# glacierbliss/iceberg_tracking_code

Measured on NVIDIA B200. Metric: tracked points/sec (24MP frame pairs, 20k pts, LK fwd+bwd+FB), higher is better.
Workload: dtype u8/int32 fixed point + f32 2x2 solve

## Files before the change

### iceberg_tracking_code_b200/csrc/common.cuh

```cuda
#pragma once
#include <cuda.h>
#include <cuda_runtime.h>
#include <stdint.h>
#include "../../include/ibt.h"

#define IBT_API extern "C" __attribute__((visibility("default")))

namespace ibt {

void set_last_error(cudaError_t e, const char *where);

inline int check_launch(const char *where)
{
    cudaError_t e = cudaGetLastError();
    if (e != cudaSuccess) { set_last_error(e, where); return IBT_E_CUDA; }
    return IBT_OK;
}

#define IBT_CUDA_TRY(expr)                                                        \
    do {                                                                          \
        cudaError_t e__ = (expr);                                                 \
        if (e__ != cudaSuccess) { ::ibt::set_last_error(e__, #expr); return IBT_E_CUDA; } \
    } while (0)

__host__ __device__ __noinline__ inline int r101_far(int i, int n)
{
    if (n == 1) return 0;
    const int p = 2 * (n - 1);
    i %= p;
    if (i < 0) i += p;
    return i < n ? i : p - i;
}
__host__ __device__ __forceinline__ int r101(int i, int n)
{
    if (i >= 0 && i < n) return i;
    if (i < 0) i = -i;
    if (i < n) return i;
    const int j = 2 * (n - 1) - i;
    if (j >= 0) return j;
    return r101_far(i, n);
}

#ifndef IBT_MBAR_SOFT
#define IBT_MBAR_SOFT 0
#endif
__device__ __forceinline__ void mbar_init(uint64_t *bar, int count)
{
    asm volatile("mbarrier.init.shared::cta.b64 [%0], %1;" ::"r"((unsigned)__cvta_generic_to_shared(bar)), "r"(count) : "memory");
}
__device__ __forceinline__ void mbar_expect_tx(uint64_t *bar, unsigned bytes)
{
    asm volatile("mbarrier.arrive.expect_tx.shared::cta.b64 _, [%0], %1;" ::"r"((unsigned)__cvta_generic_to_shared(bar)), "r"(bytes)
                 : "memory");
}
__device__ __forceinline__ void mbar_wait(uint64_t *bar, unsigned parity)
{
    const unsigned addr = (unsigned)__cvta_generic_to_shared(bar);
    for (int spin = 0; spin < (1 << 26); spin++) {
        unsigned ok;
        asm volatile("{\n .reg .pred p;\n mbarrier.try_wait.parity.shared::cta.b64 p, [%1], %2;\n selp.u32 %0, 1, 0, p;\n}"
                     : "=r"(ok) : "r"(addr), "r"(parity) : "memory");
        if (ok) return;
    }
    if (IBT_MBAR_SOFT) return;
    __trap();
}
__device__ __forceinline__ void tma_load_2d(void *smem_dst, const CUtensorMap *tmap, int c0, int c1, uint64_t *bar)
{
    asm volatile("cp.async.bulk.tensor.2d.shared::cluster.global.mbarrier::complete_tx::bytes [%0], [%1, {%2, %3}], [%4];"
                 ::"r"((unsigned)__cvta_generic_to_shared(smem_dst)), "l"(reinterpret_cast<uint64_t>(tmap)), "r"(c0), "r"(c1),
                 "r"((unsigned)__cvta_generic_to_shared(bar)) : "memory");
}
__device__ __forceinline__ void tma_prefetch_map(const CUtensorMap *tmap)
{
    asm volatile("prefetch.tensormap [%0];" ::"l"(reinterpret_cast<uint64_t>(tmap)) : "memory");
}
__device__ __forceinline__ void fence_proxy_async() { asm volatile("fence.proxy.async.shared::cta;" ::: "memory"); }

typedef CUresult (*EncodeTiledFn)(CUtensorMap *, CUtensorMapDataType, cuuint32_t, void *, const cuuint64_t *, const cuuint64_t *,
                                  const cuuint32_t *, const cuuint32_t *, CUtensorMapInterleave, CUtensorMapSwizzle,
                                  CUtensorMapL2promotion, CUtensorMapFloatOOBfill);
inline EncodeTiledFn encode_tiled_fn()
{
    static const EncodeTiledFn fn = [] {
        void *p = nullptr;
        cudaDriverEntryPointQueryResult q;
        EncodeTiledFn f = nullptr;
        if (cudaGetDriverEntryPoint("cuTensorMapEncodeTiled", &p, cudaEnableDefault, &q) == cudaSuccess &&
            q == cudaDriverEntryPointSuccess)
            f = reinterpret_cast<EncodeTiledFn>(p);
        (void)cudaGetLastError();
        return f;
    }();
    return fn;
}
inline bool make_map_2d(CUtensorMap *m, CUtensorMapDataType dt, const void *base, int cols, int rows, int64_t pitch_bytes,
                        int box_cols, int box_rows)
{
    EncodeTiledFn fn = encode_tiled_fn();
    if (!fn || reinterpret_cast<uintptr_t>(base) % 16 != 0 || pitch_bytes % 16 != 0 || box_cols > 256 || box_rows > 256) return false;
    const cuuint64_t gdim[2] = {(cuuint64_t)cols, (cuuint64_t)rows};
    const cuuint64_t gstride[1] = {(cuuint64_t)pitch_bytes};
    const cuuint32_t box[2] = {(cuuint32_t)box_cols, (cuuint32_t)box_rows};
    const cuuint32_t estr[2] = {1, 1};
    return fn(m, dt, 2, const_cast<void *>(base), gdim, gstride, box, estr, CU_TENSOR_MAP_INTERLEAVE_NONE,
              CU_TENSOR_MAP_SWIZZLE_NONE, CU_TENSOR_MAP_L2_PROMOTION_L2_128B, CU_TENSOR_MAP_FLOAT_OOB_FILL_NONE) == CUDA_SUCCESS;
}

__device__ __forceinline__ void pdl_wait() { asm volatile("griddepcontrol.wait;" ::: "memory"); }
__device__ __forceinline__ void pdl_launch_dependents() { asm volatile("griddepcontrol.launch_dependents;" ::: "memory"); }
template <typename... KArgs, typename... Args>
inline cudaError_t launch_pdl(void (*kernel)(KArgs...), dim3 grid, dim3 block, size_t smem, cudaStream_t st, Args... args)
{
    cudaLaunchConfig_t cfg = {};
    cfg.gridDim = grid; cfg.blockDim = block; cfg.dynamicSmemBytes = smem; cfg.stream = st;
    cudaLaunchAttribute attr[1];
    attr[0].id = cudaLaunchAttributeProgrammaticStreamSerialization;
    attr[0].val.programmaticStreamSerializationAllowed = 1;
// ... 37 lines not shown
```

### iceberg_tracking_code_b200/csrc/lk.cu

```cuda
#include "common.cuh"
#include <stdlib.h>
#include <string.h>
#include <type_traits>
#include <mutex>
#include <vector>

namespace ibt {

constexpr int LK_MARGIN = 3;

__host__ __device__ constexpr int lk_nl(int w) { return (w + 3) / 4; }
__host__ __device__ constexpr int lk_tcols(int w) { return 4 * lk_nl(w); }
__host__ __device__ constexpr int lk_ng0(int w, int h) { return (32 / lk_nl(w)) < h ? (32 / lk_nl(w)) : h; }
__host__ __device__ constexpr int lk_rg(int w, int h) { return (h + lk_ng0(w, h) - 1) / lk_ng0(w, h); }
__host__ __device__ constexpr int lk_ng(int w, int h) { return (h + lk_rg(w, h) - 1) / lk_rg(w, h); }
__host__ __device__ constexpr int lk_trows(int w, int h) { return lk_ng(w, h) * lk_rg(w, h); }
__host__ __device__ constexpr int lk_nstrips(int w) { return (lk_tcols(w) + 31) / 32; }
__host__ __device__ constexpr int lk_strip_cols(int w) { return (lk_tcols(w) + lk_nstrips(w) - 1) / lk_nstrips(w); }
__host__ __device__ constexpr bool lk_split(int w) { return w == 35; }
__host__ __device__ constexpr int lk_reach(int w) { return lk_split(w) ? lk_tcols(w) + 1 : (lk_nstrips(w) - 1) * lk_strip_cols(w) + 33; }
__host__ __device__ constexpr int lk_dpitch(int w) { return (lk_reach(w) + 6) & ~3; }
__host__ __device__ constexpr int lk_ipitch(int w) { return (15 + lk_reach(w) + 15) & ~15; }
__host__ __device__ constexpr int lk_jpitch(int w) { return (15 + 2 * LK_MARGIN + lk_tcols(w) + 4 + 15) & ~15; }

// ... 43 lines not shown
};

__device__ __forceinline__ long long warp_sum_wide(int v)
{
    const int lo = __reduce_add_sync(0xffffffffu, v & 0xffff);
    const int hi = __reduce_add_sync(0xffffffffu, v >> 16);
    return ((long long)hi << 16) + lo;
}

__device__ __forceinline__ int cv_floor(float v) { return __float2int_rd(v); }
__device__ __forceinline__ float no_nan(float v) { return v == v ? v : __int_as_float(0xff800000); }

__device__ __forceinline__ uint32_t dp2a_lo(uint32_t a, uint32_t b, uint32_t c)
{
    int d;
    asm("dp2a.lo.s32.u32 %0, %1, %2, %3;" : "=r"(d) : "r"(a), "r"(b), "r"((int)c));
    return (uint32_t)d;
}
__device__ __forceinline__ uint32_t dp2a_hi(uint32_t a, uint32_t b, uint32_t c)
{
    int d;
    asm("dp2a.hi.s32.u32 %0, %1, %2, %3;" : "=r"(d) : "r"(a), "r"(b), "r"((int)c));
    return (uint32_t)d;
}

__device__ __forceinline__ unsigned smem_u32(const void *p) { return (unsigned)__cvta_generic_to_shared(p); }
__device__ __forceinline__ void cp_async4(unsigned smem_dst, const void *gsrc)
{
    asm volatile("cp.async.ca.shared.global [%0], [%1], 4;" ::"r"(smem_dst), "l"(gsrc) : "memory");
}
__device__ __forceinline__ void cp_async4_zfill(unsigned smem_dst, const void *gsrc, int src_size)
{
    asm volatile("cp.async.ca.shared.global [%0], [%1], 4, %2;" ::"r"(smem_dst), "l"(gsrc), "r"(src_size) : "memory");
}
__device__ __forceinline__ void cp_async_commit() { asm volatile("cp.async.commit_group;" ::: "memory"); }
template <int N>
__device__ __forceinline__ void cp_async_wait() { asm volatile("cp.async.wait_group %0;" ::"n"(N) : "memory"); }

__device__ __forceinline__ void bilinear_weights(float a, float b, uint32_t &wtop, uint32_t &wbot,
                                                 int &iw00, int &iw01, int &iw10, int &iw11)
{
    const float oa = __fsub_rn(1.f, a), ob = __fsub_rn(1.f, b);
    iw00 = __float2int_rn(__fmul_rn(__fmul_rn(oa, ob), 16384.f));
    iw01 = __float2int_rn(__fmul_rn(__fmul_rn(a, ob), 16384.f));
    iw10 = __float2int_rn(__fmul_rn(__fmul_rn(oa, b), 16384.f));
    iw11 = 16384 - iw00 - iw01 - iw10;
    wtop = ((uint32_t)iw00 & 0xffffu) | ((uint32_t)iw01 << 16);
    wbot = ((uint32_t)iw10 & 0xffffu) | ((uint32_t)iw11 << 16);
}

__device__ __forceinline__ bool window_oob(int ix, int iy, int winW, int winH, int rows, int cols)
{
    return ix < -winW || ix >= cols || iy < -winH || iy >= rows;
}

__device__ __noinline__ void stage_bytes_border(const LKLevel &L, int x0a, int y0, int nrows, int pitch, uint8_t *dst, int lane)
{
    for (int c = lane; c < pitch; c += 32) {
        const uint8_t *s = L.img + r101(x0a + c, L.cols);
        uint8_t *d = dst + c;
        int r = 0;
        for (; r + 4 <= nrows; r += 4) {
            const uint8_t v0 = __ldg(s + (int64_t)r101(y0 + r, L.rows) * L.img_pitch);
            const uint8_t v1 = __ldg(s + (int64_t)r101(y0 + r + 1, L.rows) * L.img_pitch);
            const uint8_t v2 = __ldg(s + (int64_t)r101(y0 + r + 2, L.rows) * L.img_pitch);
            const uint8_t v3 = __ldg(s + (int64_t)r101(y0 + r + 3, L.rows) * L.img_pitch);
            d[r * pitch] = v0; d[(r + 1) * pitch] = v1; d[(r + 2) * pitch] = v2; d[(r + 3) * pitch] = v3;
        }
        for (; r < nrows; r++) d[r * pitch] = __ldg(s + (int64_t)r101(y0 + r, L.rows) * L.img_pitch);
    }
}

__device__ __forceinline__ void stage_bytes(const LKLevel &L, int x0a, int y0, int nrows, int pitch, int lane, uint8_t *dst)
{
    const bool interior = L.word_ok && x0a >= 0 && y0 >= 0 && y0 + nrows <= L.rows && x0a + pitch <= L.cols;
    if (interior) {
        const int ppw = pitch >> 2;
        const int rpp = 32 / ppw;
        const int sr = lane / ppw, sw = lane - sr * ppw;
        if (sr < rpp) {
            const uint8_t *src = L.img + (int64_t)(y0 + sr) * L.img_pitch + x0a + 4 * sw;
            unsigned d = smem_u32(dst) + sr * pitch + 4 * sw;
            const int64_t sstep = (int64_t)rpp * L.img_pitch;
            const int dstep = rpp * pitch;
#pragma unroll 4
            for (int r = sr; r < nrows; r += rpp) {
                cp_async4(d, src);
                src += sstep; d += dstep;
            }
        }
    } else {
        stage_bytes_border(L, x0a, y0, nrows, pitch, dst, lane);
    }
}

__device__ __forceinline__ bool patch_reflectable(int nx0, int nx1, int y0, int nrows, int rows, int cols)
{
    const int y1 = y0 + nrows - 1;
    return -nx0 <= nx1 && -nx0 < cols && 2 * (cols - 1) - nx1 >= nx0 && 2 * (cols - 1) - nx1 >= 0 &&
           -y0 <= y1 && -y0 < rows && 2 * (rows - 1) - y1 >= y0 && 2 * (rows - 1) - y1 >= 0;
}
__device__ __noinline__ void patch_reflect(uint8_t *patch, int pitch, int x0a, int nx0, int nx1, int y0, int nrows, int rows,
                                           int cols, int lane)
{
    __syncwarp();
    const int pw = pitch >> 2;
// ... 160 lines not shown
        a11[s] = a12[s] = a22[s] = c1[s] = c2[s] = 0;
        ipair[s] = 0; d00x[s] = d00y[s] = d01x[s] = d01y[s] = 0;
        const bool active = s < nstrips && lane < SC && s * SC + lane < winW;
        mtop[s] = active ? wtop : 0u; mbot[s] = active ? wbot : 0u;
        m00[s] = active ? iw00 : 0; m01[s] = active ? iw01 : 0; m10[s] = active ? iw10 : 0; m11[s] = active ? iw11 : 0;
        if (s < nstrips) {
            const uint8_t *ip = ip0 + s * SC + lane;
            const uint32_t *dp = dp0 + s * SC + lane;
            ipair[s] = (uint32_t)ip[0] | ((uint32_t)ip[1] << 8);
            const uint32_t dc = dp[0], dcr = dp[1];
            d00x[s] = (int)(short)(dc & 0xffffu); d00y[s] = (int)dc >> 16;
            d01x[s] = (int)(short)(dcr & 0xffffu); d01y[s] = (int)dcr >> 16;
        }
    }
#pragma unroll 4
    for (int r = 0; r < winH; r++) {
#pragma unroll
        for (int s = 0; s < NS; s++) {
            if (s < nstrips) {
                const int col = s * SC + lane;
                const uint8_t *ip = ip0 + (r + 1) * IP + col;
                const uint32_t *dp = dp0 + (r + 1) * DP + col;
                const uint32_t cpair = (uint32_t)ip[0] | ((uint32_t)ip[1] << 8);
                const uint32_t dc = dp[0], dcr = dp[1];
                const int d10x = (int)(short)(dc & 0xffffu), d10y = (int)dc >> 16;
                const int d11x = (int)(short)(dcr & 0xffffu), d11y = (int)dcr >> 16;
                uint32_t v = dp2a_lo(mtop[s], ipair[s], 256u);
                v = dp2a_lo(mbot[s], cpair, v);
                const int Iw = (int)(v >> 9);
                const int Ix = (d00x[s] * m00[s] + d01x[s] * m01[s] + d10x * m10[s] + d11x * m11[s] + 8192) >> 14;
                const int Iy = (d00y[s] * m00[s] + d01y[s] * m01[s] + d10y * m10[s] + d11y * m11[s] + 8192) >> 14;
                if ((SC >= 32 || lane < SC) && (NS * SC <= TC || col < TC))
                    tmpl_store(tmpl, r, TC, col, Ix, Iy);
                a11[s] += Ix * Ix; a12[s] += Ix * Iy; a22[s] += Iy * Iy;
                c1[s] += Iw * Ix; c2[s] += Iw * Iy;
                ipair[s] = cpair; d00x[s] = d10x; d00y[s] = d10y; d01x[s] = d11x; d01y[s] = d11y;
            }
        }
        __syncwarp();
    }
    for (int i = winH * TC + lane; i < TR * TC; i += 32) tmpl[i] = 0u;
    sA11 = sA12 = sA22 = sC1 = sC2 = 0;
#pragma unroll
    for (int s = 0; s < NS; s++) {
        if (s < nstrips) {
            sA11 += warp_sum_wide(a11[s]); sA12 += warp_sum_wide(a12[s]); sA22 += warp_sum_wide(a22[s]);
            sC1 += warp_sum_wide(c1[s]); sC2 += warp_sum_wide(c2[s]);
        }
    }
    __syncwarp();
}

template <int WW, int WH>
__device__ __forceinline__ void newton_sums(const LKArgs &a, const uint8_t *__restrict__ patch, int ox, int oy, uint32_t wtop,
                                            uint32_t wbot, const uint32_t *__restrict__ tmpl, int rowbase, int cq, bool lane_on,
                                            long long &S1, long long &S2)
{
    const int RG = (WW && WH) ? lk_rg(WW, WH) : a.rg;
    const int JP = WW ? lk_jpitch(WW) : a.jpitch, TC = WW ? lk_tcols(WW) : a.tcols;
    const uint32_t al = (uint32_t)ox & 3u;
    const uint32_t sel0 = 0x3210u + 0x1111u * al, sel1 = sel0 + 0x1111u;
    const uint32_t *jp = reinterpret_cast<const uint32_t *>(patch + (oy + rowbase) * JP + ((ox + 4 * cq) & ~3));
    const uint4 *tp = reinterpret_cast<const uint4 *>(tmpl + rowbase * TC + 4 * cq);
    uint32_t p0, p1;
    {
        const uint32_t w0 = jp[0], w1 = jp[1];
        p0 = __byte_perm(w0, w1, sel0); p1 = __byte_perm(w0, w1, sel1);
    }
    S1 = 0; S2 = 0;
    for (int r0 = 0; r0 < RG; r0 += 16) {
        const int r1 = (WW && WH) ? ((RG < r0 + 16) ? RG : r0 + 16) : min(RG, r0 + 16);
        uint32_t b1lo = 0, b1hi = 0, b2lo = 0, b2hi = 0;
#pragma unroll((WW && WH) ? 16 : 2)
        for (int r = r0; r < r1; r++) {
            jp += JP >> 2;
            const uint32_t w0 = jp[0], w1 = jp[1];
            const uint32_t c0 = __byte_perm(w0, w1, sel0), c1 = __byte_perm(w0, w1, sel1);
            const uint4 t = tp[r * (TC >> 2)];
            const uint32_t j0 = dp2a_lo(wbot, c0, dp2a_lo(wtop, p0, 256u)) >> 9;
            const uint32_t j1 = dp2a_lo(wbot, c1, dp2a_lo(wtop, p1, 256u)) >> 9;
            const uint32_t j2 = dp2a_hi(wbot, c0, dp2a_hi(wtop, p0, 256u)) >> 9;
            const uint32_t j3 = dp2a_hi(wbot, c1, dp2a_hi(wtop, p1, 256u)) >> 9;
            const uint32_t jb01 = __byte_perm(j0, j1, 0x5140u), jb23 = __byte_perm(j2, j3, 0x5140u);
            b1lo = dp2a_lo(t.y, jb23, dp2a_lo(t.x, jb01, b1lo));
            b1hi = dp2a_hi(t.y, jb23, dp2a_hi(t.x, jb01, b1hi));
            b2lo = dp2a_lo(t.w, jb23, dp2a_lo(t.z, jb01, b2lo));
            b2hi = dp2a_hi(t.w, jb23, dp2a_hi(t.z, jb01, b2hi));
            p0 = c0; p1 = c1;
        }
        if (!lane_on) { b1lo = b1hi = b2lo = b2hi = 0; }
        S1 += (long long)__reduce_add_sync(0xffffffffu, (int)b1lo) + ((long long)__reduce_add_sync(0xffffffffu, (int)b1hi) << 8);
        S2 += (long long)__reduce_add_sync(0xffffffffu, (int)b2lo) + ((long long)__reduce_add_sync(0xffffffffu, (int)b2hi) << 8);
    }
}

template <int WW, int WH>
__device__ __noinline__ long long window_err(const LKArgs &a, const uint8_t *jpatch, int ox, int oy, uint32_t wtop, uint32_t wbot,
                                             const uint8_t *ipatch, int iox, uint32_t iwtop, uint32_t iwbot, int rowbase, int cq,
                                             bool lane_on)
{
    const int winW = WW ? WW : a.winW, winH = WH ? WH : a.winH;
    const int RG = (WW && WH) ? lk_rg(WW, WH) : a.rg;
    const int JP = WW ? lk_jpitch(WW) : a.jpitch, IP = WW ? lk_ipitch(WW) : a.ipitch;
    const uint32_t jsel0 = 0x3210u + 0x1111u * ((uint32_t)ox & 3u), jsel1 = jsel0 + 0x1111u;
    const uint32_t isel0 = 0x3210u + 0x1111u * ((uint32_t)iox & 3u), isel1 = isel0 + 0x1111u;
    const uint32_t *jp = reinterpret_cast<const uint32_t *>(jpatch + (oy + rowbase) * JP + ((ox + 4 * cq) & ~3));
    const uint32_t *ip = reinterpret_cast<const uint32_t *>(ipatch + rowbase * IP + ((iox + 4 * cq) & ~3));
    uint32_t jp0 = __byte_perm(jp[0], jp[1], jsel0), jp1 = __byte_perm(jp[0], jp[1], jsel1);
    uint32_t ip0 = __byte_perm(ip[0], ip[1], isel0), ip1 = __byte_perm(ip[0], ip[1], isel1);
    long long S = 0;
    for (int r0 = 0; r0 < RG; r0 += 16) {
        int s = 0;
        for (int r = r0; r < min(RG, r0 + 16); r++) {
            jp += JP >> 2; ip += IP >> 2;
            const uint32_t jc0 = __byte_perm(jp[0], jp[1], jsel0), jc1 = __byte_perm(jp[0], jp[1], jsel1);
            const uint32_t ic0 = __byte_perm(ip[0], ip[1], isel0), ic1 = __byte_perm(ip[0], ip[1], isel1);
            if (rowbase + r < winH) {
                const int d0 = (int)(dp2a_lo(wbot, jc0, dp2a_lo(wtop, jp0, 256u)) >> 9) - (int)(dp2a_lo(iwbot, ic0, dp2a_lo(iwtop, ip0, 256u)) >> 9);
                const int d1 = (int)(dp2a_lo(wbot, jc1, dp2a_lo(wtop, jp1, 256u)) >> 9) - (int)(dp2a_lo(iwbot, ic1, dp2a_lo(iwtop, ip1, 256u)) >> 9);
                const int d2 = (int)(dp2a_hi(wbot, jc0, dp2a_hi(wtop, jp0, 256u)) >> 9) - (int)(dp2a_hi(iwbot, ic0, dp2a_hi(iwtop, ip0, 256u)) >> 9);
                const int d3 = (int)(dp2a_hi(wbot, jc1, dp2a_hi(wtop, jp1, 256u)) >> 9) - (int)(dp2a_hi(iwbot, ic1, dp2a_hi(iwtop, ip1, 256u)) >> 9);
                const int c = 4 * cq;
                if (c < winW) s += abs(d0);
                if (c + 1 < winW) s += abs(d1);
                if (c + 2 < winW) s += abs(d2);
                if (c + 3 < winW) s += abs(d3);
            }
            jp0 = jc0; jp1 = jc1; ip0 = ic0; ip1 = ic1;
        }
        if (!lane_on) s = 0;
        S += warp_sum_wide(s);
    }
    return S;
}

template <typename T>
__device__ __forceinline__ T *lk_chan(T *p, int c, int stride)
{
    using B = std::conditional_t<std::is_const<T>::value, const unsigned char, unsigned char>;
    return reinterpret_cast<T *>(reinterpret_cast<B *>(p) + (size_t)c * stride);
}

template <int WW, int WH, int CN>
__device__ __forceinline__ void lk_point(const LKPyr *PI, const LKPyr *PJ, int cn_rt, const LKArgs &a, float ptx, float pty,
                                         bool use_init, bool want_status, bool want_err, float &ox, float &oy, int &status,
                                         float &err, int &iters, unsigned char *slab, int rowbase, int cq, bool lane_on,
                                         int lane, const CUtensorMap *mapI, const CUtensorMap *mapJ, const CUtensorMap *mapD,
                                         uint64_t *bars, unsigned &phases)
{
    const float FLT_SCALE = 1.f / (1 << 20);
    const int cn = CN ? CN : cn_rt;
    const int winW = WW ? WW : a.winW, winH = WH ? WH : a.winH;
    const int IPITCH = WW ? lk_ipitch(WW) : a.ipitch, JPITCH = WW ? lk_jpitch(WW) : a.jpitch;
    const int DPITCH = WW ? lk_dpitch(WW) : a.dpitch;
    const int JROWS = winH + 1 + 2 * LK_MARGIN;
    const float halfx = (winW - 1) * 0.5f, halfy = (winH - 1) * 0.5f;
    uint32_t *tmpl = reinterpret_cast<uint32_t *>(slab);
    uint32_t *dpatch = reinterpret_cast<uint32_t *>(slab);
    uint8_t *ipatch = slab + a.off_ipatch;
    uint8_t *jpatch = slab + a.off_jpatch;
    auto ch = [&](auto *p, int c) { return lk_chan(p, c, a.warp_smem); };
    auto chl = [](const LKLevel &l, int c) -> const LKLevel & { return *lk_chan(&l, c, (int)sizeof(LKPyr)); };
    status = 1; err = 0.f;
    const int L = PI[0].nlevels;
    for (int level = L - 1; level >= 0; --level) {
        const LKLevel &LI = PI[0].lv[level];
        const LKLevel &LJ = PJ[0].lv[level];
        const int rows = LI.rows, cols = LI.cols;
        const float sc = __int_as_float((127 - level) << 23);
        float ppx = __fmul_rn(ptx, sc), ppy = __fmul_rn(pty, sc);
        float nx, ny;
        if (level == L - 1) {
            if (use_init) { nx = __fmul_rn(ox, sc); ny = __fmul_rn(oy, sc); }
            else { nx = ppx; ny = ppy; }
        } else { nx = __fmul_rn(ox, 2.f); ny = __fmul_rn(oy, 2.f); }
        ox = nx; oy = ny;

        ppx = __fsub_rn(ppx, halfx); ppy = __fsub_rn(ppy, halfy);
        const int ipx = cv_floor(no_nan(ppx)), ipy = cv_floor(no_nan(ppy));
        if (window_oob(ipx, ipy, winW, winH, rows, cols)) {
            if (level == 0) { status = 0; err = 0.f; }
            continue;
        }
        nx = no_nan(__fsub_rn(nx, halfx)); ny = no_nan(__fsub_rn(ny, halfy));

        const bool i_in = ipx >= 0 && ipy >= 0 && ipx + winW < cols && ipy + winH < rows;
        const bool i_fix = !i_in && patch_reflectable(ipx, ipx + winW, ipy, winH + 1, rows, cols);
        const bool i_tma = LI.tma_img && (i_in || i_fix), d_tma = LI.tma_der != 0;
        const int ipxa = i_tma ? (ipx & ~15) : (ipx & ~3);
        const int doff = d_tma ? (ipx & 3) : 0;
        int px0 = 0, py0 = 0, vx0 = 0;
        bool staged = false, j_tma = false, j_fix = false;
        const int jnx = cv_floor(nx), jny = cv_floor(ny);
        const bool j_ok = !window_oob(jnx, jny, winW, winH, rows, cols);
        if (j_ok) {
            const int bx = jnx - LK_MARGIN, by = jny - LK_MARGIN;
            const bool j_in = bx >= 0 && by >= 0 && bx + winW + 2 * LK_MARGIN < cols && by + JROWS <= rows;
            j_fix = !j_in && patch_reflectable(bx, bx + winW + 2 * LK_MARGIN, by, JROWS, rows, cols);
            j_tma = LJ.tma_img && (j_in || j_fix);
            px0 = j_tma ? (bx & ~15) : (bx & ~3); py0 = by; vx0 = bx;
            staged = true;
        }
        if (lane == 0 && (i_tma || d_tma || j_tma)) {
            fence_proxy_async();
            if (i_tma || d_tma) {
                mbar_expect_tx(&bars[0], (i_tma ? (unsigned)(IPITCH * (winH + 1)) : 0u) + (d_tma ? (unsigned)(DPITCH * 4 * (winH + 1)) : 0u));
                if (i_tma) tma_load_2d(ipatch, &mapI[level], ipxa, ipy, &bars[0]);
                if (d_tma) tma_load_2d(dpatch, &mapD[level], ipx - doff, ipy, &bars[0]);
            }
            if (j_tma) {
                mbar_expect_tx(&bars[1], (unsigned)(JPITCH * JROWS));
                tma_load_2d(jpatch, &mapJ[level], px0, py0, &bars[1]);
            }
        }
        for (int c = 0; c < cn; c++) {
            if (!i_tma) stage_bytes(chl(LI, c), ipxa, ipy, winH + 1, IPITCH, lane, ch(ipatch, c));
            if (!d_tma) stage_deriv<WW, WH>(chl(LI, c), a, ipx, ipy, ch(dpatch, c), lane);
        }
        cp_async_commit();
        if (j_ok && !j_tma)
            for (int c = 0; c < cn; c++) stage_bytes(chl(LJ, c), px0, py0, JROWS, JPITCH, lane, ch(jpatch, c));
        cp_async_commit();
        cp_async_wait<1>();
        if (i_tma || d_tma) { mbar_wait(&bars[0], phases & 1u); phases ^= 1u; }
        __syncwarp();
        if (i_tma && i_fix) patch_reflect(ipatch, IPITCH, ipxa, ipx, ipx + winW, ipy, winH + 1, rows, cols, lane);

        uint32_t wtop, wbot;
        int iw00, iw01, iw10, iw11;
        bilinear_weights(__fsub_rn(ppx, (float)ipx), __fsub_rn(ppy, (float)ipy), wtop, wbot, iw00, iw01, iw10, iw11);
        const uint32_t iwtop = wtop, iwbot = wbot;

        long long sA11, sA12, sA22, sC1, sC2;
        build_template<WW, WH>(a, ipatch + (ipx - ipxa), dpatch + doff, tmpl, wtop, wbot, iw00, iw01, iw10, iw11, lane,
                               sA11, sA12, sA22, sC1, sC2);
        for (int c = 1; c < cn; c++) {
            long long t11, t12, t22, tc1, tc2;
            build_template<WW, WH>(a, ch(ipatch, c) + (ipx - ipxa), ch(dpatch, c) + doff, ch(tmpl, c), wtop, wbot, iw00, iw01, iw10, iw11, lane,
                                   t11, t12, t22, tc1, tc2);
            sA11 += t11; sA12 += t12; sA22 += t22; sC1 += tc1; sC2 += tc2;
        }
        cp_async_wait<0>();
        if (j_tma) { mbar_wait(&bars[1], (phases >> 1) & 1u); phases ^= 2u; }
        __syncwarp();
        if (j_tma && j_fix) patch_reflect(jpatch, JPITCH, px0, vx0, vx0 + winW + 2 * LK_MARGIN, py0, JROWS, rows, cols, lane);
        const float A11 = __fmul_rn(__ll2float_rn(sA11), FLT_SCALE);
        const float A12 = __fmul_rn(__ll2float_rn(sA12), FLT_SCALE);
        const float A22 = __fmul_rn(__ll2float_rn(sA22), FLT_SCALE);
        float D = __fsub_rn(__fmul_rn(A11, A22), __fmul_rn(A12, A12));
        const float dA = __fsub_rn(A11, A22);
        const float disc = __fadd_rn(__fmul_rn(dA, dA), __fmul_rn(__fmul_rn(4.f, A12), A12));
        const float minEig = __fdiv_rn(__fsub_rn(__fadd_rn(A22, A11), __fsqrt_rn(disc)), (float)(2 * winW * winH));
        if (a.flags & IBT_LK_GET_MIN_EIGENVALS) err = minEig;
        if (minEig < a.minEigThr || D < 1.1920929e-07f) {
            if (level == 0) status = 0;
            continue;
        }
        D = __fdiv_rn(1.f, D);
        float pdx = 0.f, pdy = 0.f;
        for (int j = 0; j < a.maxCount; j++) {
            const int inx = cv_floor(nx), iny = cv_floor(ny);
            if (window_oob(inx, iny, winW, winH, rows, cols)) {
                if (level == 0) status = 0;
                break;
            }
            if (!staged || (unsigned)(inx - vx0) > 2u * LK_MARGIN || (unsigned)(iny - py0) > 2u * LK_MARGIN) {
                vx0 = inx - LK_MARGIN; px0 = vx0 & ~3; py0 = iny - LK_MARGIN;
                for (int c = 0; c < cn; c++) restage_sync(chl(LJ, c), px0, py0, JROWS, JPITCH, ch(jpatch, c), lane);
                staged = true;
            }
            bilinear_weights(__fsub_rn(nx, (float)inx), __fsub_rn(ny, (float)iny), wtop, wbot, iw00, iw01, iw10, iw11);
            long long sb1 = 0, sb2 = 0;
            for (int c = 0; c < cn; c++) {
                long long t1, t2;
                newton_sums<WW, WH>(a, ch(jpatch, c), inx - px0, iny - py0, wtop, wbot, ch(tmpl, c), rowbase, cq, lane_on, t1, t2);
                sb1 += t1; sb2 += t2;
            }
            ++iters;
            const float b1 = __fmul_rn(__ll2float_rn(sb1 - sC1), FLT_SCALE);
            const float b2 = __fmul_rn(__ll2float_rn(sb2 - sC2), FLT_SCALE);
            const float dx = __fmul_rn(__fsub_rn(__fmul_rn(A12, b2), __fmul_rn(A22, b1)), D);
            const float dy = __fmul_rn(__fsub_rn(__fmul_rn(A12, b1), __fmul_rn(A11, b2)), D);
            nx = __fadd_rn(nx, dx); ny = __fadd_rn(ny, dy);
            ox = __fadd_rn(nx, halfx); oy = __fadd_rn(ny, halfy);
            if (__fadd_rn(__fmul_rn(dx, dx), __fmul_rn(dy, dy)) <= a.eps2) break;
            if (j > 0 && fabsf(__fadd_rn(dx, pdx)) < 0.01f && fabsf(__fadd_rn(dy, pdy)) < 0.01f) {
                ox = __fsub_rn(ox, __fmul_rn(dx, 0.5f)); oy = __fsub_rn(oy, __fmul_rn(dy, 0.5f));
                break;
            }
            pdx = dx; pdy = dy;
        }
        if (status && level == 0 && !(a.flags & IBT_LK_GET_MIN_EIGENVALS) && (want_status || want_err)) {
            const float qx = __fsub_rn(ox, halfx), qy = __fsub_rn(oy, halfy);
            const int iqx = cv_floor(no_nan(qx)), iqy = cv_floor(no_nan(qy));
            if (window_oob(iqx, iqy, winW, winH, rows, cols)) { status = 0; err = 0.f; continue; }
            if (!want_err) continue;
            if (!staged || (unsigned)(iqx - vx0) > 2u * LK_MARGIN || (unsigned)(iqy - py0) > 2u * LK_MARGIN) {
                vx0 = iqx - LK_MARGIN; px0 = vx0 & ~3; py0 = iqy - LK_MARGIN;
                for (int c = 0; c < cn; c++) restage_sync(chl(LJ, c), px0, py0, JROWS, JPITCH, ch(jpatch, c), lane);
            }
            bilinear_weights(__fsub_rn(qx, (float)iqx), __fsub_rn(qy, (float)iqy), wtop, wbot, iw00, iw01, iw10, iw11);
            long long s = 0;
            for (int c = 0; c < cn; c++)
                s += window_err<WW, WH>(a, ch(jpatch, c), iqx - px0, iqy - py0, wtop, wbot, ch(ipatch, c), ipx - ipxa, iwtop, iwbot,
                                        rowbase, cq, lane_on);
            err = __fdiv_rn(__ll2float_rn(s), (float)(32 * winW * cn * winH));
        }
        __syncwarp();
    }
    cp_async_wait<0>();
    if (!status && !(a.flags & IBT_LK_GET_MIN_EIGENVALS)) err = 0.f;
}

template <int CN> using LKFrames = std::conditional_t<CN == 1, LKMaps, LKMcPyr>;

template <int WW, int WH, int CN>
__global__ void __launch_bounds__(256, CN == 1 ? 3 : 0)
lk_kernel(const __grid_constant__ LKArgs a, const __grid_constant__ LKFrames<CN> fr)
{
    extern __shared__ __align__(128) unsigned char lk_smem[];
    __shared__ __align__(8) uint64_t lk_bars[8][2];
    const int lane = threadIdx.x & 31, wib = threadIdx.x >> 5;
    if (lane == 0) {
        mbar_init(&lk_bars[wib][0], 1); mbar_init(&lk_bars[wib][1], 1);
        asm volatile("fence.mbarrier_init.release.cluster;" ::: "memory");
    }
    __syncwarp();
    unsigned phases = 0u;
    int cn = 1;
    if constexpr (CN != 1) cn = fr.cn;
    unsigned char *slab = lk_smem + (size_t)wib * a.warp_smem * cn;
    const int NL = WW ? lk_nl(WW) : a.nl, NG = (WW && WH) ? lk_ng(WW, WH) : a.ng, RG = (WW && WH) ? lk_rg(WW, WH) : a.rg;
    const int grp = lane / NL;
    const bool lane_on = grp < NG;
    const int rowbase = lane_on ? grp * RG : 0, cq = lane_on ? lane - grp * NL : 0;

  for (;;) {
    int k = 0;
    if (lane == 0) k = (int)atomicAdd(a.work_counter, 1u);
    k = __shfl_sync(0xffffffffu, k, 0);
    if (k >= a.n) break;
    if (a.alive && !a.alive[k]) continue;
    const float p0x = a.p0[2 * k], p0y = a.p0[2 * k + 1];
    float ptx = p0x, pty = p0y;
    int it_f = 0, it_b = 0;
    const int npass = a.fb ? 2 : 1;
    for (int pass = 0; pass < npass; ++pass) {
        float ox = 0.f, oy = 0.f, err;
        int status, iters = 0;
        const bool use_init = pass == 0 && (a.flags & IBT_LK_USE_INITIAL_FLOW) != 0;
        if (use_init) { ox = a.p1[2 * k]; oy = a.p1[2 * k + 1]; }
        const bool want_status = pass == 0 ? a.st1 != nullptr : a.st0 != nullptr;
        const bool want_err = pass == 0 ? a.err1 != nullptr : a.err0 != nullptr;
        const LKPyr *PI = a.pyr + pass, *PJ = a.pyr + (pass ^ 1);
        const CUtensorMap *mapI = nullptr, *mapJ = nullptr, *mapD = nullptr;
        if constexpr (CN == 1) { mapI = fr.imgI[pass]; mapJ = fr.imgJ[pass ^ 1]; mapD = fr.der[pass]; }
        else { PI = pass ? fr.J : fr.I; PJ = pass ? fr.I : fr.J; }
        lk_point<WW, WH, CN>(PI, PJ, cn, a, ptx, pty, use_init, want_status, want_err, ox, oy, status, err, iters,
                             slab, rowbase, cq, lane_on, lane, mapI, mapJ, mapD, lk_bars[wib], phases);
        if (pass == 0) it_f = iters; else it_b = iters;
        if (lane == 0) {
            if (pass == 0) {
                a.p1[2 * k] = ox; a.p1[2 * k + 1] = oy;
                if (a.st1) a.st1[k] = (uint8_t)status;
                if (a.err1) a.err1[k] = err;
            } else {
                if (a.p0r) { a.p0r[2 * k] = ox; a.p0r[2 * k + 1] = oy; }
                if (a.st0) a.st0[k] = (uint8_t)status;
                if (a.err0) a.err0[k] = err;
                const float d = hypotf(fabsf(__fsub_rn(p0x, ox)), fabsf(__fsub_rn(p0y, oy)));
                if (a.fbdist) a.fbdist[k] = d;
                if (a.alive) a.alive[k] = (d < a.fb_thresh) ? 1 : 0;
            }
        }
        ptx = ox; pty = oy;
    }
    if (lane == 0) {
        if (a.iters) {
            if (a.fb) { a.iters[2 * k] = it_f; a.iters[2 * k + 1] = it_b; }
            else a.iters[k] = it_f;
        }
        if (a.iter_total) atomicAdd(a.iter_total, (unsigned long long)(it_f + it_b));
    }
    __syncwarp();
  }
    if (lane == 0) {
        __threadfence();
        if (atomicAdd(a.work_counter + 1, 1u) == a.total_warps - 1u) {
            a.work_counter[0] = 0u; a.work_counter[1] = 0u;
            __threadfence();
        }
    }
}

static int fill_pyr(const ibt_pyramid_t *p, LKPyr &o, bool need_deriv)
{
    if (!p || p->nlevels < 1 || p->nlevels > IBT_MAX_LEVELS) return IBT_E_INVALID;
    o.nlevels = p->nlevels;
    for (int l = 0; l < p->nlevels; l++) {
        if (!p->img[l] || p->rows[l] <= 0 || p->cols[l] <= 0 || p->img_pitch[l] < p->cols[l] ||
            p->img_pitch[l] > 0x7fffffff)
            return IBT_E_INVALID;
        if (need_deriv && (!p->deriv[l] || p->deriv_pitch[l] % 4 != 0 || p->deriv_pitch[l] < (int64_t)p->cols[l] * 4 ||
                           reinterpret_cast<uintptr_t>(p->deriv[l]) % 4 != 0))
            return IBT_E_INVALID;
        o.lv[l].img = p->img[l];
        o.lv[l].deriv = reinterpret_cast<const uint32_t *>(p->deriv[l]);
        o.lv[l].img_pitch = (int)p->img_pitch[l];
        o.lv[l].deriv_pitch = (int)(p->deriv_pitch[l] / 4);
        o.lv[l].rows = p->rows[l];
        o.lv[l].cols = p->cols[l];
        o.lv[l].word_ok = (reinterpret_cast<uintptr_t>(p->img[l]) % 4 == 0) && (p->img_pitch[l] % 4 == 0);
        o.lv[l].tma_img = o.lv[l].tma_der = 0;
    }
    return IBT_OK;
}

struct LKQueue { int dev; cudaStream_t stream; unsigned int *words; };
static std::mutex lk_mu;
static int lk_max_ctas_per_sm = 0;
static std::vector<LKQueue> lk_queues;
static bool lk_attr_set[64] = {false};

static int lk_queue_for(int dev, cudaStream_t st, unsigned int **out)
{
    for (const LKQueue &q : lk_queues)
        if (q.dev == dev && q.stream == st) { *out = q.words; return IBT_OK; }
    unsigned int *w = nullptr;
    IBT_CUDA_TRY(cudaMalloc(&w, 2 * sizeof(unsigned int)));
    IBT_CUDA_TRY(cudaMemsetAsync(w, 0, 2 * sizeof(unsigned int), st));
    lk_queues.push_back({dev, st, w});
    *out = w;
    return IBT_OK;
}

static int launch_lk(LKArgs &a, const ibt_pyramid_t *const *A, const ibt_pyramid_t *const *B, int cn, bool planes, int winW,
                     int winH, int max_count, double epsilon, double min_eig, cudaStream_t st)
{
// ... 51 lines not shown
    if (epsilon > 10) epsilon = 10;
    a.eps2 = (float)(epsilon * epsilon);
    a.minEigThr = (float)min_eig;
    const size_t per_warp = (size_t)a.warp_smem * cn;
    const int max_warps = planes ? 16 : 24;
    int wpc = 1, best = 0, best_ctas = 1;
    for (int w = 1; w <= 8; w++) {
        const size_t per_cta = per_warp * w + 1024;
        if (per_cta > 200 * 1024) break;
        int ctas = (int)((227 * 1024) / per_cta);
        if (ctas > 32) ctas = 32;
        if (ctas * w > max_warps) ctas = max_warps / w;
        const int warps = ctas * w;
        if (warps >= best) { best = warps; wpc = w; best_ctas = ctas; }
    }
    if (best == 0) return IBT_E_INVALID;
    {
        std::lock_guard<std::mutex> lock(lk_mu);
        if (lk_max_ctas_per_sm > 0 && best_ctas > lk_max_ctas_per_sm) best_ctas = lk_max_ctas_per_sm;
    }
    const size_t smem = per_warp * wpc;
    void (*kern)(const LKArgs, const LKMaps) = lk_kernel<0, 0, 1>;
    if (winW == 21 && winH == 21) kern = lk_kernel<21, 21, 1>;
    else if (winW == 31 && winH == 31) kern = lk_kernel<31, 31, 1>;
    else if (winW == 35 && winH == 35) kern = lk_kernel<35, 35, 1>;
    int dev_id = 0;
    IBT_CUDA_TRY(cudaGetDevice(&dev_id));
    if (dev_id < 0 || dev_id >= 64) return IBT_E_INVALID;
    {
        std::lock_guard<std::mutex> lock(lk_mu);
        if (!lk_attr_set[dev_id]) {
            const int lim = 200 * 1024;
            IBT_CUDA_TRY(cudaFuncSetAttribute(lk_kernel<0, 0, 1>, cudaFuncAttributeMaxDynamicSharedMemorySize, lim));
            IBT_CUDA_TRY(cudaFuncSetAttribute(lk_kernel<21, 21, 1>, cudaFuncAttributeMaxDynamicSharedMemorySize, lim));
            IBT_CUDA_TRY(cudaFuncSetAttribute(lk_kernel<31, 31, 1>, cudaFuncAttributeMaxDynamicSharedMemorySize, lim));
            IBT_CUDA_TRY(cudaFuncSetAttribute(lk_kernel<35, 35, 1>, cudaFuncAttributeMaxDynamicSharedMemorySize, lim));
            IBT_CUDA_TRY(cudaFuncSetAttribute(lk_kernel<0, 0, 0>, cudaFuncAttributeMaxDynamicSharedMemorySize, lim));
            lk_attr_set[dev_id] = true;
        }
        const int rc = lk_queue_for(dev_id, st, &a.work_counter);
        if (rc) return rc;
    }
    int blocks = kNumSMs * best_ctas;
    const int need = (a.n + wpc - 1) / wpc;
    if (blocks > need) blocks = need;
    a.total_warps = (unsigned)(blocks * wpc);
    if (planes) lk_kernel<0, 0, 0><<<blocks, wpc * 32, smem, st>>>(a, mc);
    else kern<<<blocks, wpc * 32, smem, st>>>(a, maps);
    return check_launch(planes ? "ibt_lk_multichannel" : "ibt_lk");
}

}

IBT_API int ibt_lk_set_max_ctas_per_sm(int ctas)
{
    if (ctas < 0) return IBT_E_INVALID;
    std::lock_guard<std::mutex> lock(ibt::lk_mu);
    ibt::lk_max_ctas_per_sm = ctas;
    return IBT_OK;
}

IBT_API int ibt_lk(const ibt_pyramid_t *pyrI, const ibt_pyramid_t *pyrJ, const float *pts, float *next_pts, int N,
                   int winW, int winH, int max_count, double epsilon, double min_eig_threshold, int flags,
                   uint8_t *status, float *err, int32_t *iters, void *stream)
{
    ibt::LKArgs a;
    memset(&a, 0, sizeof(a));
    a.p0 = pts; a.n = N; a.flags = flags; a.fb = 0;
    a.p1 = next_pts; a.st1 = status; a.err1 = err; a.iters = iters;
    return ibt::launch_lk(a, &pyrI, &pyrJ, 1, false, winW, winH, max_count, epsilon, min_eig_threshold,
                          static_cast<cudaStream_t>(stream));
}

IBT_API int ibt_lk_fb(const ibt_pyramid_t *prev, const ibt_pyramid_t *next, const float *p0, int N, int winW, int winH,
                      int max_count, double epsilon, double min_eig_threshold, float fb_threshold, float *p1,
                      uint8_t *st1, float *err1, float *p0r, uint8_t *st0, float *err0, float *fbdist, uint8_t *alive,
                      int32_t *iters, unsigned long long *iter_total, void *stream)
{
    ibt::LKArgs a;
    memset(&a, 0, sizeof(a));
    a.p0 = p0; a.n = N; a.flags = 0; a.fb = 1; a.fb_thresh = fb_threshold;
    a.p1 = p1; a.st1 = st1; a.err1 = err1; a.p0r = p0r; a.st0 = st0; a.err0 = err0;
    a.fbdist = fbdist; a.alive = alive; a.iters = iters; a.iter_total = iter_total;
    return ibt::launch_lk(a, &prev, &next, 1, false, winW, winH, max_count, epsilon, min_eig_threshold,
                          static_cast<cudaStream_t>(stream));
}

IBT_API int ibt_lk_multichannel(const ibt_pyramid_t *const *pyrI, const ibt_pyramid_t *const *pyrJ, int cn, const float *pts,
                                float *next_pts, int N, int winW, int winH, int max_count, double epsilon,
                                double min_eig_threshold, int flags, uint8_t *status, float *err, int32_t *iters, void *stream)
{
    ibt::LKArgs a;
    memset(&a, 0, sizeof(a));
    a.p0 = pts; a.n = N; a.flags = flags; a.fb = 0;
    a.p1 = next_pts; a.st1 = status; a.err1 = err; a.iters = iters;
    return ibt::launch_lk(a, pyrI, pyrJ, cn, true, winW, winH, max_count, epsilon, min_eig_threshold,
                          static_cast<cudaStream_t>(stream));
}

IBT_API int ibt_lk_fb_multichannel(const ibt_pyramid_t *const *prev, const ibt_pyramid_t *const *next, int cn, const float *p0,
                                   int N, int winW, int winH, int max_count, double epsilon, double min_eig_threshold,
                                   float fb_threshold, float *p1, uint8_t *st1, float *err1, float *p0r, uint8_t *st0,
                                   float *err0, float *fbdist, uint8_t *alive, int32_t *iters, unsigned long long *iter_total,
                                   void *stream)
{
    if (cn < 2 || cn > ibt::LK_MC_MAX) return IBT_E_INVALID;
// ... 9 lines not shown
```

Before: 27.47 million.

## Skip per-iteration bounds checks when staged J patch is safe, add phase profiling

```diff
diff --git a/iceberg_tracking_code_b200/csrc/common.cuh b/iceberg_tracking_code_b200/csrc/common.cuh
--- a/iceberg_tracking_code_b200/csrc/common.cuh
+++ b/iceberg_tracking_code_b200/csrc/common.cuh
@@ -64,6 +64,20 @@
     }
     if (IBT_MBAR_SOFT) return;
     __trap();
+}
+__device__ __forceinline__ unsigned mbar_wait_parked(uint64_t *bar, unsigned parity)
+{
+    const unsigned addr = (unsigned)__cvta_generic_to_shared(bar);
+#pragma unroll 1
+    for (unsigned spin = 1; spin <= (1u << 20); spin++) {
+        unsigned ok;
+        asm volatile("{\n .reg .pred p;\n mbarrier.try_wait.parity.shared::cta.b64 p, [%1], %2, %3;\n selp.u32 %0, 1, 0, p;\n}"
+                     : "=r"(ok) : "r"(addr), "r"(parity), "r"(20000u) : "memory");
+        if (ok) return spin;
+    }
+    if (IBT_MBAR_SOFT) return 0u;
+    __trap();
+    return 0u;
 }
 __device__ __forceinline__ void tma_load_2d(void *smem_dst, const CUtensorMap *tmap, int c0, int c1, uint64_t *bar)
 {
diff --git a/iceberg_tracking_code_b200/csrc/lk.cu b/iceberg_tracking_code_b200/csrc/lk.cu
--- a/iceberg_tracking_code_b200/csrc/lk.cu
+++ b/iceberg_tracking_code_b200/csrc/lk.cu
@@ -119,6 +119,46 @@
 __device__ __forceinline__ bool window_oob(int ix, int iy, int winW, int winH, int rows, int cols)
 {
     return ix < -winW || ix >= cols || iy < -winH || iy >= rows;
+}
+__device__ __forceinline__ bool lk_box_in_bounds(int x0, int y0, int winW, int winH, int rows, int cols)
+{
+    return x0 >= -winW && x0 + 2 * LK_MARGIN < cols && y0 >= -winH && y0 + 2 * LK_MARGIN < rows;
+}
+
+enum { LKP_WAIT, LKP_TEMPLATE, LKP_NEWTON, LKP_ITER, LKP_LEVEL, LKP_POINT, LKP_N, LKP_POLLS = LKP_N, LKP_SLOTS };
+#ifndef IBT_LK_PHASES
+#define IBT_LK_PHASES 0
+#endif
+#if IBT_LK_PHASES
+__device__ unsigned long long lk_phase_cycles[LKP_SLOTS];
+struct LKPhaseClock {
+    unsigned long long *row;
+    unsigned t;
+    __device__ __forceinline__ void start(unsigned long long *r) { row = r; t = (unsigned)clock(); }
+    __device__ __forceinline__ void to(int phase)
+    {
+        const unsigned n = (unsigned)clock();
+        if ((threadIdx.x & 31) == 0) row[phase] += n - t;
+        t = n;
+    }
+    __device__ __forceinline__ void polls(unsigned k) { if ((threadIdx.x & 31) == 0) row[LKP_POLLS] += k; }
+};
+#else
+struct LKPhaseClock {
+    __device__ __forceinline__ void start(unsigned long long *) {}
+    __device__ __forceinline__ void to(int) {}
+    __device__ __forceinline__ void polls(unsigned) {}
+};
+#endif
+
+template <int WW, int WH>
+__device__ __forceinline__ void lk_newton_lane(const LKArgs &a, int lane, int &rowbase, int &cq, bool &lane_on)
+{
+    const int NL = WW ? lk_nl(WW) : a.nl, NG = (WW && WH) ? lk_ng(WW, WH) : a.ng, RG = (WW && WH) ? lk_rg(WW, WH) : a.rg;
+    const int grp = lane / NL;
+    lane_on = grp < NG;
+    rowbase = lane_on ? grp * RG : 0;
+    cq = lane_on ? lane - grp * NL : 0;
 }
 
 __device__ __noinline__ void stage_bytes_border(const LKLevel &L, int x0a, int y0, int nrows, int pitch, uint8_t *dst, int lane)
@@ -385,22 +425,23 @@
 }
 
 template <int WW, int WH>
-__device__ __forceinline__ void newton_sums(const LKArgs &a, const uint8_t *__restrict__ patch, int ox, int oy, uint32_t wtop,
-                                            uint32_t wbot, const uint32_t *__restrict__ tmpl, int rowbase, int cq, bool lane_on,
-                                            long long &S1, long long &S2)
+__device__ __forceinline__ void newton_sums(const LKArgs &a, const uint8_t *__restrict__ jlane, int ox, int oy, uint32_t wtop,
+                                            uint32_t wbot, const uint32_t *__restrict__ tlane, bool lane_on,
+                                            long long &S1, long long &S2, LKPhaseClock &pc)
 {
     const int RG = (WW && WH) ? lk_rg(WW, WH) : a.rg;
     const int JP = WW ? lk_jpitch(WW) : a.jpitch, TC = WW ? lk_tcols(WW) : a.tcols;
     const uint32_t al = (uint32_t)ox & 3u;
     const uint32_t sel0 = 0x3210u + 0x1111u * al, sel1 = sel0 + 0x1111u;
-    const uint32_t *jp = reinterpret_cast<const uint32_t *>(patch + (oy + rowbase) * JP + ((ox + 4 * cq) & ~3));
-    const uint4 *tp = reinterpret_cast<const uint4 *>(tmpl + rowbase * TC + 4 * cq);
+    const uint32_t *jp = reinterpret_cast<const uint32_t *>(jlane + oy * JP + (ox & ~3));
+    const uint4 *tp = reinterpret_cast<const uint4 *>(tlane);
     uint32_t p0, p1;
     {
         const uint32_t w0 = jp[0], w1 = jp[1];
         p0 = __byte_perm(w0, w1, sel0); p1 = __byte_perm(w0, w1, sel1);
     }
     S1 = 0; S2 = 0;
+    pc.to(LKP_ITER);
     for (int r0 = 0; r0 < RG; r0 += 16) {
         const int r1 = (WW && WH) ? ((RG < r0 + 16) ? RG : r0 + 16) : min(RG, r0 + 16);
         uint32_t b1lo = 0, b1hi = 0, b2lo = 0, b2hi = 0;
@@ -421,6 +462,7 @@
             b2hi = dp2a_hi(t.w, jb23, dp2a_hi(t.z, jb01, b2hi));
             p0 = c0; p1 = c1;
         }
+        pc.to(LKP_NEWTON);
         if (!lane_on) { b1lo = b1hi = b2lo = b2hi = 0; }
         S1 += (long long)__reduce_add_sync(0xffffffffu, (int)b1lo) + ((long long)__reduce_add_sync(0xffffffffu, (int)b1hi) << 8);
         S2 += (long long)__reduce_add_sync(0xffffffffu, (int)b2lo) + ((long long)__reduce_add_sync(0xffffffffu, (int)b2hi) << 8);
@@ -429,9 +471,11 @@
 
 template <int WW, int WH>
 __device__ __noinline__ long long window_err(const LKArgs &a, const uint8_t *jpatch, int ox, int oy, uint32_t wtop, uint32_t wbot,
-                                             const uint8_t *ipatch, int iox, uint32_t iwtop, uint32_t iwbot, int rowbase, int cq,
-                                             bool lane_on)
-{
+                                             const uint8_t *ipatch, int iox, uint32_t iwtop, uint32_t iwbot, int lane)
+{
+    int rowbase, cq;
+    bool lane_on;
+    lk_newton_lane<WW, WH>(a, lane, rowbase, cq, lane_on);
     const int winW = WW ? WW : a.winW, winH = WH ? WH : a.winH;
     const int RG = (WW && WH) ? lk_rg(WW, WH) : a.rg;
     const int JP = WW ? lk_jpitch(WW) : a.jpitch, IP = WW ? lk_ipitch(WW) : a.ipitch;
@@ -477,9 +521,9 @@
 template <int WW, int WH, int CN>
 __device__ __forceinline__ void lk_point(const LKPyr *PI, const LKPyr *PJ, int cn_rt, const LKArgs &a, float ptx, float pty,
                                          bool use_init, bool want_status, bool want_err, float &ox, float &oy, int &status,
-                                         float &err, int &iters, unsigned char *slab, int rowbase, int cq, bool lane_on,
-                                         int lane, const CUtensorMap *mapI, const CUtensorMap *mapJ, const CUtensorMap *mapD,
-                                         uint64_t *bars, unsigned &phases)
+                                         float &err, int &iters, unsigned char *slab, int jl, int tl, bool lane_on,
+                                         int lane, const LKMaps *maps, int pass,
+                                         uint64_t *bars, unsigned &phases, LKPhaseClock &pc)
 {
     const float FLT_SCALE = 1.f / (1 << 20);
     const int cn = CN ? CN : cn_rt;
@@ -496,6 +540,7 @@
     auto chl = [](const LKLevel &l, int c) -> const LKLevel & { return *lk_chan(&l, c, (int)sizeof(LKPyr)); };
     status = 1; err = 0.f;
     const int L = PI[0].nlevels;
+    pc.to(LKP_POINT);
     for (int level = L - 1; level >= 0; --level) {
         const LKLevel &LI = PI[0].lv[level];
         const LKLevel &LJ = PJ[0].lv[level];
@@ -538,12 +583,12 @@
             fence_proxy_async();
             if (i_tma || d_tma) {
                 mbar_expect_tx(&bars[0], (i_tma ? (unsigned)(IPITCH * (winH + 1)) : 0u) + (d_tma ? (unsigned)(DPITCH * 4 * (winH + 1)) : 0u));
-                if (i_tma) tma_load_2d(ipatch, &mapI[level], ipxa, ipy, &bars[0]);
-                if (d_tma) tma_load_2d(dpatch, &mapD[level], ipx - doff, ipy, &bars[0]);
+                if (i_tma) tma_load_2d(ipatch, &maps->imgI[pass][level], ipxa, ipy, &bars[0]);
+                if (d_tma) tma_load_2d(dpatch, &maps->der[pass][level], ipx - doff, ipy, &bars[0]);
             }
             if (j_tma) {
                 mbar_expect_tx(&bars[1], (unsigned)(JPITCH * JROWS));
-                tma_load_2d(jpatch, &mapJ[level], px0, py0, &bars[1]);
+                tma_load_2d(jpatch, &maps->imgJ[pass ^ 1][level], px0, py0, &bars[1]);
             }
         }
         for (int c = 0; c < cn; c++) {
@@ -554,9 +599,11 @@
         if (j_ok && !j_tma)
             for (int c = 0; c < cn; c++) stage_bytes(chl(LJ, c), px0, py0, JROWS, JPITCH, lane, ch(jpatch, c));
         cp_async_commit();
+        pc.to(LKP_LEVEL);
         cp_async_wait<1>();
-        if (i_tma || d_tma) { mbar_wait(&bars[0], phases & 1u); phases ^= 1u; }
+        if (i_tma || d_tma) { pc.polls(mbar_wait_parked(&bars[0], phases & 1u)); phases ^= 1u; }
         __syncwarp();
+        pc.to(LKP_WAIT);
         if (i_tma && i_fix) patch_reflect(ipatch, IPITCH, ipxa, ipx, ipx + winW, ipy, winH + 1, rows, cols, lane);
 
         uint32_t wtop, wbot;
@@ -565,6 +612,7 @@
         const uint32_t iwtop = wtop, iwbot = wbot;
 
         long long sA11, sA12, sA22, sC1, sC2;
+        pc.to(LKP_LEVEL);
         build_template<WW, WH>(a, ipatch + (ipx - ipxa), dpatch + doff, tmpl, wtop, wbot, iw00, iw01, iw10, iw11, lane,
                                sA11, sA12, sA22, sC1, sC2);
         for (int c = 1; c < cn; c++) {
@@ -573,9 +621,11 @@
                                    t11, t12, t22, tc1, tc2);
             sA11 += t11; sA12 += t12; sA22 += t22; sC1 += tc1; sC2 += tc2;
         }
+        pc.to(LKP_TEMPLATE);
         cp_async_wait<0>();
-        if (j_tma) { mbar_wait(&bars[1], (phases >> 1) & 1u); phases ^= 2u; }
+        if (j_tma) { pc.polls(mbar_wait_parked(&bars[1], (phases >> 1) & 1u)); phases ^= 2u; }
         __syncwarp();
+        pc.to(LKP_WAIT);
         if (j_tma && j_fix) patch_reflect(jpatch, JPITCH, px0, vx0, vx0 + winW + 2 * LK_MARGIN, py0, JROWS, rows, cols, lane);
         const float A11 = __fmul_rn(__ll2float_rn(sA11), FLT_SCALE);
         const float A12 = __fmul_rn(__ll2float_rn(sA12), FLT_SCALE);
@@ -591,22 +641,27 @@
         }
         D = __fdiv_rn(1.f, D);
         float pdx = 0.f, pdy = 0.f;
+        bool jsafe = staged && lk_box_in_bounds(vx0, py0, winW, winH, rows, cols);
+        pc.to(LKP_LEVEL);
         for (int j = 0; j < a.maxCount; j++) {
             const int inx = cv_floor(nx), iny = cv_floor(ny);
-            if (window_oob(inx, iny, winW, winH, rows, cols)) {
-                if (level == 0) status = 0;
-                break;
-            }
-            if (!staged || (unsigned)(inx - vx0) > 2u * LK_MARGIN || (unsigned)(iny - py0) > 2u * LK_MARGIN) {
-                vx0 = inx - LK_MARGIN; px0 = vx0 & ~3; py0 = iny - LK_MARGIN;
-                for (int c = 0; c < cn; c++) restage_sync(chl(LJ, c), px0, py0, JROWS, JPITCH, ch(jpatch, c), lane);
-                staged = true;
+            if (!(jsafe && (unsigned)(inx - vx0) <= 2u * LK_MARGIN && (unsigned)(iny - py0) <= 2u * LK_MARGIN)) {
+                if (window_oob(inx, iny, winW, winH, rows, cols)) {
+                    if (level == 0) status = 0;
+                    break;
+                }
+                if (!staged || (unsigned)(inx - vx0) > 2u * LK_MARGIN || (unsigned)(iny - py0) > 2u * LK_MARGIN) {
+                    vx0 = inx - LK_MARGIN; px0 = vx0 & ~3; py0 = iny - LK_MARGIN;
+                    for (int c = 0; c < cn; c++) restage_sync(chl(LJ, c), px0, py0, JROWS, JPITCH, ch(jpatch, c), lane);
+                    staged = true;
+                }
+                jsafe = lk_box_in_bounds(vx0, py0, winW, winH, rows, cols);
             }
             bilinear_weights(__fsub_rn(nx, (float)inx), __fsub_rn(ny, (float)iny), wtop, wbot, iw00, iw01, iw10, iw11);
             long long sb1 = 0, sb2 = 0;
             for (int c = 0; c < cn; c++) {
                 long long t1, t2;
-                newton_sums<WW, WH>(a, ch(jpatch, c), inx - px0, iny - py0, wtop, wbot, ch(tmpl, c), rowbase, cq, lane_on, t1, t2);
+                newton_sums<WW, WH>(a, ch(jpatch + jl, c), inx - px0, iny - py0, wtop, wbot, ch(tmpl + tl, c), lane_on, t1, t2, pc);
                 sb1 += t1; sb2 += t2;
             }
             ++iters;
@@ -623,6 +678,7 @@
             }
             pdx = dx; pdy = dy;
         }
+        pc.to(LKP_ITER);
         if (status && level == 0 && !(a.flags & IBT_LK_GET_MIN_EIGENVALS) && (want_status || want_err)) {
             const float qx = __fsub_rn(ox, halfx), qy = __fsub_rn(oy, halfy);
             const int iqx = cv_floor(no_nan(qx)), iqy = cv_floor(no_nan(qy));
@@ -636,7 +692,7 @@
             long long s = 0;
             for (int c = 0; c < cn; c++)
                 s += window_err<WW, WH>(a, ch(jpatch, c), iqx - px0, iqy - py0, wtop, wbot, ch(ipatch, c), ipx - ipxa, iwtop, iwbot,
-                                        rowbase, cq, lane_on);
+                                        lane);
             err = __fdiv_rn(__ll2float_rn(s), (float)(32 * winW * cn * winH));
         }
         __syncwarp();
@@ -663,10 +719,22 @@
     int cn = 1;
     if constexpr (CN != 1) cn = fr.cn;
     unsigned char *slab = lk_smem + (size_t)wib * a.warp_smem * cn;
-    const int NL = WW ? lk_nl(WW) : a.nl, NG = (WW && WH) ? lk_ng(WW, WH) : a.ng, RG = (WW && WH) ? lk_rg(WW, WH) : a.rg;
-    const int grp = lane / NL;
-    const bool lane_on = grp < NG;
-    const int rowbase = lane_on ? grp * RG : 0, cq = lane_on ? lane - grp * NL : 0;
+    int jl, tl;
+    bool lane_on;
+    {
+        int rowbase, cq;
+        lk_newton_lane<WW, WH>(a, lane, rowbase, cq, lane_on);
+        jl = rowbase * (WW ? lk_jpitch(WW) : a.jpitch) + 4 * cq;
+        tl = rowbase * (WW ? lk_tcols(WW) : a.tcols) + 4 * cq;
+    }
+    LKPhaseClock pc;
+#if IBT_LK_PHASES
+    __shared__ unsigned long long lk_phase_row[8][LKP_SLOTS];
+    if (lane == 0)
+        for (int p = 0; p < LKP_SLOTS; p++) lk_phase_row[wib][p] = 0ull;
+    __syncwarp();
+    pc.start(lk_phase_row[wib]);
+#endif
 
   for (;;) {
     int k = 0;
@@ -676,7 +744,7 @@
     if (a.alive && !a.alive[k]) continue;
     const float p0x = a.p0[2 * k], p0y = a.p0[2 * k + 1];
     float ptx = p0x, pty = p0y;
-    int it_f = 0, it_b = 0;
+    int it_sum = 0;
     const int npass = a.fb ? 2 : 1;
     for (int pass = 0; pass < npass; ++pass) {
         float ox = 0.f, oy = 0.f, err;
@@ -686,13 +754,14 @@
         const bool want_status = pass == 0 ? a.st1 != nullptr : a.st0 != nullptr;
         const bool want_err = pass == 0 ? a.err1 != nullptr : a.err0 != nullptr;
         const LKPyr *PI = a.pyr + pass, *PJ = a.pyr + (pass ^ 1);
-        const CUtensorMap *mapI = nullptr, *mapJ = nullptr, *mapD = nullptr;
-        if constexpr (CN == 1) { mapI = fr.imgI[pass]; mapJ = fr.imgJ[pass ^ 1]; mapD = fr.der[pass]; }
+        const LKMaps *maps = nullptr;
+        if constexpr (CN == 1) maps = &fr;
         else { PI = pass ? fr.J : fr.I; PJ = pass ? fr.I : fr.J; }
         lk_point<WW, WH, CN>(PI, PJ, cn, a, ptx, pty, use_init, want_status, want_err, ox, oy, status, err, iters,
-                             slab, rowbase, cq, lane_on, lane, mapI, mapJ, mapD, lk_bars[wib], phases);
-        if (pass == 0) it_f = iters; else it_b = iters;
+                             slab, jl, tl, lane_on, lane, maps, pass, lk_bars[wib], phases, pc);
+        it_sum += iters;
         if (lane == 0) {
+            if (a.iters) a.iters[a.fb ? 2 * k + pass : k] = iters;
             if (pass == 0) {
                 a.p1[2 * k] = ox; a.p1[2 * k + 1] = oy;
                 if (a.st1) a.st1[k] = (uint8_t)status;
@@ -708,15 +777,14 @@
         }
         ptx = ox; pty = oy;
     }
-    if (lane == 0) {
-        if (a.iters) {
-            if (a.fb) { a.iters[2 * k] = it_f; a.iters[2 * k + 1] = it_b; }
-            else a.iters[k] = it_f;
-        }
-        if (a.iter_total) atomicAdd(a.iter_total, (unsigned long long)(it_f + it_b));
-    }
+    if (lane == 0 && a.iter_total) atomicAdd(a.iter_total, (unsigned long long)it_sum);
     __syncwarp();
+    pc.to(LKP_POINT);
   }
+#if IBT_LK_PHASES
+    if (lane == 0)
+        for (int p = 0; p < LKP_SLOTS; p++) atomicAdd(&lk_phase_cycles[p], lk_phase_row[wib][p]);
+#endif
     if (lane == 0) {
         __threadfence();
         if (atomicAdd(a.work_counter + 1, 1u) == a.total_warps - 1u) {
@@ -874,6 +942,19 @@
 
 }
 
+#if IBT_LK_PHASES
+IBT_API int ibt_lk_phase_cycles(unsigned long long *out, int reset)
+{
+    IBT_CUDA_TRY(cudaDeviceSynchronize());
+    IBT_CUDA_TRY(cudaMemcpyFromSymbol(out, ibt::lk_phase_cycles, sizeof(ibt::lk_phase_cycles)));
+    if (reset) {
+        static const unsigned long long zero[ibt::LKP_SLOTS] = {};
+        IBT_CUDA_TRY(cudaMemcpyToSymbol(ibt::lk_phase_cycles, zero, sizeof(zero)));
+    }
+    return IBT_OK;
+}
+#endif
+
 IBT_API int ibt_lk_set_max_ctas_per_sm(int ctas)
 {
     if (ctas < 0) return IBT_E_INVALID;
```

New measurement: 28.19 million (median of 6 runs). 1.03x the previous value.
